# ssskkkky/EMME

Hardware: AMD Instinct MI355X
Metric: omega-points solved/sec (256-pt grid) (higher is better)
Workload: dtype f64

## Files before the change

### emme_amd/_lib.py

```python
from __future__ import annotations

import ctypes as C
import os

import numpy as np

HERE = os.path.dirname(os.path.abspath(__file__))
_LIB = None


class EmmeError(RuntimeError):
    def __init__(self, code, msg):
        super().__init__(f"[emme {code}] {msg}")
        self.code = code
        self.reason = msg


def lib_path() -> str:
    return os.environ.get("EMME_LIB") or os.path.join(HERE, "libemme_hip.so")


class Params(C.Structure):

    _fields_ = [
# ... 126 lines not shown
    lib.emme_ctx_set_options.argtypes = [P, C.POINTER(Options)]
    lib.emme_ctx_get_options.argtypes = [P, C.POINTER(Options)]
    lib.emme_null_vectors_batch.argtypes = [P, C.c_int, C.c_int, P, P, P]
    lib.emme_ctx_destroy.argtypes = [P]
    lib.emme_ctx_destroy.restype = None
    lib.emme_release_pooled_memory.argtypes = []
    lib.emme_release_pooled_memory.restype = None
    lib.emme_ctx_set_stream.argtypes = [P, P]
    lib.emme_ctx_set_tile_shapes.argtypes = [P, C.c_int]
    lib.emme_ctx_get_tile_shapes.argtypes = [P]
    lib.emme_ctx_set_deriv_cache_shapes.argtypes = [P, C.c_int]
    lib.emme_ctx_get_deriv_cache_shapes.argtypes = [P]
    if hasattr(lib, "emme_ctx_set_mirror_pairs"):
        lib.emme_ctx_set_mirror_pairs.argtypes = [P, C.c_int]
        lib.emme_ctx_get_mirror_pairs.argtypes = [P]
    lib.emme_ctx_dim.argtypes = [P]
    lib.emme_ctx_fill_mode.argtypes = [P]
    lib.emme_ctx_last_deferred.argtypes = [P]
    lib.emme_ctx_last_deferred.restype = C.c_longlong
    lib.emme_ctx_node_cache_gib.argtypes = [P]
    lib.emme_ctx_node_cache_gib.restype = C.c_double
    lib.emme_ctx_cache_settle.argtypes = [P, P, C.c_int, P]
    lib.emme_ctx_cache_state.argtypes = [P, P, P, P]
    lib.emme_ctx_profile_enable.argtypes = [P, C.c_int]
    lib.emme_ctx_profile_read.argtypes = [P, C.POINTER(Profile), C.c_int]
    lib.emme_assemble_batch.argtypes = [P, P, C.c_int, P, P]
    lib.emme_trace_solve_batch.argtypes = [P, C.c_int, C.c_int, P, P, P, P]
    lib.emme_qr_secant_batch.argtypes = [P, C.c_int, C.c_int, P, P, P, P]
    lib.emme_newton_step_batch.argtypes = [P, P, P, C.c_int, P, P, C.c_int, P]
    lib.emme_solve_roots.argtypes = [P, P, C.c_int, C.c_double, C.c_int, P, P, P, P]
# ... 364 lines not shown
    first = next((h for h in host if h is not None), None)
    nb, n = (first.shape[0], first.shape[1]) if first is not None else (int(A[0]), int(A[1]))
    for h in host:
        if h is not None and h.shape != (nb, n, n):
            raise ValueError("the operands must be [nbatch, n, n] of one shape")
    ptrs = [h.ctypes.data if h is not None else C.c_void_p(p) for h, p in zip(host, (a_device_ptr, b_device_ptr))]
    return ptrs[0], ptrs[1], nb, n, host


class Context:

    def __init__(self, params: Params, device: int = -1, **options):
        self.lib = load()
        self.params = params
        h = C.c_void_p()
        o = default_options(**options)
        _check(self.lib.emme_ctx_create_ex(C.byref(params), device, C.byref(o), C.byref(h)))
        self.h = h
        self.dim = self.lib.emme_ctx_dim(h)

    def options(self) -> Options:
        o = Options()
        _check(self.lib.emme_ctx_get_options(self.h, C.byref(o)))
        return o

    def set_options(self, **kw) -> None:
        o = self.options()
        for k, v in kw.items():
            if not hasattr(o, k):
                raise TypeError(f"unknown option {k!r}")
            setattr(o, k, v)
        _check(self.lib.emme_ctx_set_options(self.h, C.byref(o)))

    def set_tile_shapes(self, shapes: int) -> None:
# ... 4 lines not shown

    def deriv_cache_shapes(self) -> int:
        v = self.lib.emme_ctx_get_deriv_cache_shapes(self.h)
        if v < 0:
            _check(v)
        return v

    def tile_shapes(self) -> int:
        v = self.lib.emme_ctx_get_tile_shapes(self.h)
        if v < 0:
            _check(v)
        return v

    def set_mirror_pairs(self, on: bool) -> None:
        _check(self.lib.emme_ctx_set_mirror_pairs(self.h, 1 if on else 0))

    def mirror_pairs(self) -> int:
        v = self.lib.emme_ctx_get_mirror_pairs(self.h)
        if v < 0:
            _check(v)
        return v

    def close(self):
        if getattr(self, "h", None):
            self.lib.emme_ctx_destroy(self.h)
            self.h = None

    def __del__(self):
        try:
            self.close()
# ... 573 lines not shown
```

### emme_amd/csrc/ctx.hpp

```cpp
#pragma once
#include <hip/hip_runtime.h>

#include <algorithm>
#include <chrono>
#include <cmath>
#include <cstdio>
#include <cstdlib>
#include <cstring>
#include <functional>
#include <limits>
#include <mutex>
#include <string>
#include <vector>

#include "../../include/emme_hip.h"
#include "buffers.hpp"
#include "launch.hpp"
#include "options.hpp"
#include "pair_list.hpp"
#include "step_feedback.hpp"

namespace emme {

void set_error(const std::string& msg);
// ... 68 lines not shown
    emme_options_t opt{};
    int cache_depth = -1;
    NodeCacheGeom cache_geom{};
    int cache_max_intervals = 0;
    NodeCacheClass cache[2];
    bool em_shared = false;
    bool folded = true;
    bool tiled = false;
    DeviceBuffer<> d_btab;
    DeviceBuffer<> d_etab;
    DeviceBuffer<int> d_lu_items;
    DeviceBuffer<> d_lu_scratch;
    int n_cu = 256;
    int last_lu_nwg = 1;
    bool lu_one_wg = false;
    PinnedBuffer<int> p_act;
    PinnedBuffer<unsigned long long> p_iv;
    PinnedBuffer<double> p_w;
    PinnedBuffer<unsigned int> p_deferred;
    DeviceBuffer<unsigned int> d_overflow;
    PinnedBuffer<unsigned int> p_overflow;
    emme::StepFeedback fb;
    emme::StagingRing lists;
    bool ext_failed = false;
    DeviceBuffer<unsigned long long> d_defer_info;
    double cache_bytes_used = 0.0;
    DeviceBuffer<double> d_scale;
    DeviceBuffer<unsigned long long> d_worklist;
    DeviceBuffer<unsigned int> d_worklist_count;
    DeviceBuffer<unsigned long long> d_tile_worklist;
// ... 75 lines not shown
inline size_t batch_bytes(int n, int nbatch) { return (size_t)n * n * 2 * sizeof(double) * nbatch; }
int check_set_indices(const emme_ctx* c, const int* set, int n, const char* who);
int upload_set_indices(emme_ctx* c, const int* set, int n);
int ensure_batch(emme_ctx* c, int nb);
int ensure_mats(emme_ctx* c, int nb, int sets);
int upload_omega(emme_ctx* c, const double* omega, int n, hipMemcpyKind kind = hipMemcpyHostToDevice);
int reset_fill_counters(emme_ctx* c, int n);
int collect_fill_status(emme_ctx* c, int n, long long* intervals, int* bad_item = nullptr);
int queue_fill_counters(emme_ctx* c, int n, std::vector<unsigned long long>& iv, std::vector<int>* st);
int fold_fill_counters(emme_ctx* c, const std::vector<unsigned long long>& iv, const std::vector<int>* st,
                       long long* intervals = nullptr);

int check_method(const emme_ctx* c, int method);
hipError_t linear_step(emme_ctx* c, int method, int n, int nbatch, const double* M, double* work, double* Mp,
                       const int* active, double* tr, int* info, const int* h_active = nullptr, bool work_ready = false);
struct LuScratch {
    DeviceBuffer<double> b;
    DeviceBuffer<int> maps;
};
int lu_factor_batch(emme_ctx* c, int n, int nbatch, double* work, LuScratch& s, const char* who,
                    const std::function<hipError_t(int b0, int nb, const int* maps, int map_nb, const int* lu_info)>& after,
                    const int* d_items = nullptr, int nitems = 0);

struct AllocTimer {
    emme_ctx* c;
    std::chrono::steady_clock::time_point t0 = std::chrono::steady_clock::now();
    bool running = true;
    explicit AllocTimer(emme_ctx* ctx) : c(ctx) {}
    void stop() {
        if (running) {
// ... 32 lines not shown
```

### emme_amd/csrc/ctx_fill.hip

```cpp
#include "ctx.hpp"
#include "fill_plan.hpp"

namespace emme {

namespace {

FillShape shape_of(const emme_ctx* c, bool mirrored = false) {
    FillShape s;
    s.tiled = c->tiled, s.folded = c->folded;
    s.nm = c->nm, s.gk_points = c->p.integration_start_points, s.npairs = mirrored ? c->npairs_half : c->npairs;
    s.fill_lanes = c->opt.fill == EMME_FILL_LANES;
    s.dense_min_tasks = c->opt.dense_min_tasks, s.dense_cost_ratio = c->opt.dense_cost_ratio;
    s.union_ipg_few = c->opt.union_ipg_few, s.union_few_chunks = c->opt.union_few_chunks;
    return s;
}

bool deriv_shape_is_es15(const emme_ctx* c) { return c->nm == 1 && c->p.integration_start_points == 15; }
bool deriv_from_cache(const emme_ctx* c, const FillRequest& r) {
    return r.d_Md && c->opt.deriv_cached != 0 && c->tiled &&
           (deriv_shape_is_es15(c) || c->deriv_cache_shapes == EMME_DERIV_CACHE_SHAPES_ALL) && r.host_omega != nullptr;
}

bool runs_mirrored(const emme_ctx* c, const FillRequest& r, bool use_cache) {
    return c->mirror && c->tiled && use_cache && !r.d_Md && !r.d_set;
// ... 402 lines not shown
    ScopedSpan span(c, K_ASM);
    HIP_TRY((r.d_Md ? launch_assemble_sets_deriv : launch_assemble_sets)(L, c->d_sets, c->d_set_tabs, r.d_set, c->stream));
    return EMME_OK;
}

int fill_by_class(emme_ctx* c, const FillRequest& r, int minority) {
    std::vector<int> major(r.nbatch, 0), minor(r.nbatch, 0);
    for (int b : c->h_actidx) (contour_class(r.host_omega[2 * b]) == minority ? minor : major)[b] = 1;
    FillRequest part = r;
    part.host_active = major.data();
    EMME_TRY(fill(c, part));
    const int mode = c->last_fill_mode;
    part.host_active = minor.data(), part.force_uncached = true;
    const int rc = fill(c, part);
    c->last_fill_mode = mode;
    return rc;
}

}

int fill(emme_ctx* c, const FillRequest& r) {
    const bool has_wide = r.newton_loop && !r.d_Md && !r.d_set && c->tiled && c->nm == 1 && !c->fb.wide.empty();
    const int n_wide = plan_order(r.nbatch, r.host_active, r.cost, has_wide ? c->fb.wide.data() : nullptr, c->h_actidx);
    const int n_act = (int)c->h_actidx.size();
    if (n_act == 0) return EMME_OK;
    if (r.d_set) {
        AssembleLaunch L = make_launch(c, r, false);
        EMME_TRY(launch_sets(c, L, r));
        c->acc.matrices += n_act;
        return EMME_OK;
    }
    if (c->mirror && deriv_from_cache(c, r)) EMME_TRY(drop_mirror(c));
    bool use_cache = wants_cache(c, r);
    if (use_cache && !c->cache[0].recs && !c->cache[1].recs) c->mirror = mirror_wanted(c) && r.may_mirror;
    AssembleLaunch L = make_launch(c, r, runs_mirrored(c, r, use_cache));
    if (use_cache) {
        const bool has_cache[2] = {(bool)c->cache[0].recs, (bool)c->cache[1].recs};
        const ClassCensus classes = plan_classes(c->h_actidx, r.host_omega, has_cache);
        if (classes.minority >= 0) return fill_by_class(c, r, classes.minority);
        for (int k = 0; k < 2 && use_cache; ++k)
            if (classes.count[k] > 0) use_cache = ensure_node_cache(c, L, k);
        if (!use_cache && L.mirror) L = make_launch(c, r, false);
    }
    EMME_TRY(use_cache ? grow_cache_from_deferrals(c, L) : EMME_OK);
    EMME_TRY(use_cache ? fill_cached(c, L, r, n_wide) : fill_uncached(c, L, r));
    c->acc.matrices += n_act;
    return EMME_OK;
}

}
```

### emme_amd/csrc/ctx_linstep.hip

```cpp
#include "ctx.hpp"
#include "linstep_plan.hpp"

using namespace emme;

namespace {

hipError_t trace_solve(emme_ctx* c, int n, int nbatch, double* A, double* B, const int* active,
                       double* tr, int* info, const int* h_active) {
    const bool fits = trace_solve_blocked_lds(n) <= 150 * 1024;
    if (c->opt.lu_unblocked == 0 && (fits || n <= 1024)) {
        hipError_t e = c->d_lu_scratch.grow(trace_solve_blocked_scratch(n, nbatch));
        if (e != hipSuccess) return e;
        int n_live = nbatch;
        int* lu_slot = nullptr;
        if (h_active) {
            e = c->d_lu_items.grow(sizeof(int) * nbatch);
            if (e == hipSuccess) e = c->lists.take(nbatch, &lu_slot);
            if (e != hipSuccess) return e;
            n_live = 0;
            for (int b = 0; b < nbatch; ++b)
                if (h_active[b]) lu_slot[n_live++] = b;
            if (n_live == 0) return hipSuccess;
        }
        const int nwg = lu_workgroups(n, n_live, c->n_cu, c->opt.lu_split, c->lu_one_wg, fits);
// ... 46 lines not shown
    return EMME_OK;
}

hipError_t linear_step(emme_ctx* c, int method, int n, int nbatch, const double* M, double* work,
                       double* Mp, const int* active, double* tr, int* info, const int* h_active, bool work_ready) {
    if (method == EMME_METHOD_QR_SECANT) {
        hipError_t e = launch_transpose(n, nbatch, M, work, active, c->stream);
        if (e != hipSuccess) return e;
        return launch_qr_secant(n, nbatch, work, Mp, active, tr, info, c->stream);
    }
    if (!work_ready) {
        hipError_t e = hipMemcpyAsync(work, M, batch_bytes(n, nbatch), hipMemcpyDeviceToDevice, c->stream);
        if (e != hipSuccess) return e;
    }
    return trace_solve(c, n, nbatch, work, Mp, active, tr, info, h_active);
}

int lu_factor_batch(emme_ctx* c, int n, int nbatch, double* work, LuScratch& s, const char* who,
                    const std::function<hipError_t(int, int, const int*, int, const int*)>& after, const int* d_items,
                    int nitems) {
    const size_t mbytes = batch_bytes(n, 1);
    const bool one_wg = trace_solve_blocked_lds(n) <= 150 * 1024;
    const int todo = d_items ? nitems : nbatch;
    if (todo < 1) return EMME_OK;
    if (one_wg || (n <= 1024 && !(d_items && c->lu_one_wg))) {
        const int slice_max = one_wg ? todo : std::max(1, c->n_cu / 2);
        const int held = d_items ? nbatch : std::min(nbatch, slice_max);
        HIP_TRY(c->d_lu_scratch.grow(trace_solve_blocked_scratch(n, held)));
        if (!one_wg) HIP_TRY(s.b.grow(mbytes * held));
        for (int b0 = 0; b0 < todo; b0 += slice_max) {
// ... 97 lines not shown
    const size_t bytes = batch_bytes(n, nbatch);
    DeviceOperands ops;
    hipError_t staged = hipSuccess;
    EMME_TRY(ops.stage(c, A, B, bytes, &staged));
    HIP_TRY(staged);
    {
        ScopedSpan s(c, K_LIN);
        HIP_TRY(trace_solve(c, n, nbatch, ops.A, ops.B, nullptr, c->d_tr, c->d_info, nullptr));
    }
    HIP_TRY(hipMemcpyAsync(tr, c->d_tr, sizeof(double) * 2 * nbatch, hipMemcpyDeviceToHost, c->stream));
    HIP_TRY(hipMemcpyAsync(info, c->d_info, sizeof(int) * nbatch, hipMemcpyDeviceToHost, c->stream));
    HIP_TRY(hipStreamSynchronize(c->stream));
    return EMME_OK;
}

int emme_qr_secant_batch(emme_ctx_t* c, int n, int nbatch, const double* A, const double* B,
                         double* q, int* info) {
    if (!c || !A || !B || !q || !info || n < 1 || nbatch < 1) return EMME_EINVAL;
    if (n > 1024) {
        set_error("QR-secant step: matrix dimension above 1024 is not supported");
        return EMME_ECONFIG;
    }
    HIP_TRY(hipSetDevice(c->device));
    EMME_TRY(ensure_batch(c, nbatch));
    const size_t bytes = batch_bytes(n, nbatch);
    DeviceOperands ops;
    DeviceBuffer<double> dW;
    hipError_t e = hipSuccess;
    EMME_TRY(ops.stage(c, A, B, bytes, &e));
    if (e == hipErrorOutOfMemory || dW.grow(bytes) != hipSuccess) {
// ... 77 lines not shown
```

### emme_amd/csrc/ctx_search.hip

```cpp
#include "ctx.hpp"

using namespace emme;

namespace {

struct RootSearch {
    const double* guesses;
    int n;
    double tol;
    int step_limit;
    bool want_iterates;
    int method = 0;
    const int* set = nullptr;
    bool eigpair = false;
    const double* v0 = nullptr;
    LuScratch lu;
    std::vector<int> act, zeros;
    int stride() const { return step_limit + 1; }
    void to(const emme_ctx* c, FillRequest& r) const {
        if (set) r.d_set = c->d_set, r.host_set = set;
    }
    double* d_iterates(const emme_ctx* c) const { return want_iterates ? c->d_iterates.get() : nullptr; }
};

int search_begin(emme_ctx* c, RootSearch& s, int mat_sets) {
    const int n = s.n;
    EMME_TRY(ensure_batch(c, n));
    EMME_TRY(ensure_mats(c, n, mat_sets));
    if (s.want_iterates) {
        const size_t need = (size_t)n * s.stride() * 2;
        HIP_TRY(c->d_iterates.grow(need * sizeof(double)));
        std::vector<double> nanv(need, std::numeric_limits<double>::quiet_NaN());
        HIP_TRY(hipMemcpyAsync(c->d_iterates, nanv.data(), need * sizeof(double), hipMemcpyHostToDevice, c->stream));
        HIP_TRY(hipStreamSynchronize(c->stream));
    }
    s.act.assign(n, 1), s.zeros.assign(n, 0);
    if (s.set) EMME_TRY(upload_set_indices(c, s.set, n));
    if (s.eigpair) {
        const size_t vbytes = sizeof(double) * 2 * (size_t)n * c->dim;
        HIP_TRY(c->d_vecs.grow(vbytes));
        HIP_TRY(c->d_resid.grow(sizeof(double) * n));
        HIP_TRY(c->p_live.grow(sizeof(int) * n));
        if (s.v0) HIP_TRY(hipMemcpyAsync(c->d_vecs, s.v0, vbytes, hipMemcpyHostToDevice, c->stream));
    }
    HIP_TRY(hipMemcpyAsync(c->d_active, s.act.data(), sizeof(int) * n, hipMemcpyHostToDevice, c->stream));
    HIP_TRY(hipMemcpyAsync(c->d_iters, s.zeros.data(), sizeof(int) * n, hipMemcpyHostToDevice, c->stream));
    HIP_TRY(hipMemcpyAsync(c->d_info, s.zeros.data(), sizeof(int) * n, hipMemcpyHostToDevice, c->stream));
    return reset_fill_counters(c, n);
}

int search_end(emme_ctx* c, const RootSearch& s, double* roots, int* iters, int* info, double* iterates, bool* repeat) {
// ... 64 lines not shown
    StepFeedback& fb = c->fb;
    fb.begin(n);
    HIP_TRY(hipMemsetAsync(c->d_overflow, 0, sizeof(unsigned int) * n, c->stream));
    std::vector<double> h_w(2 * (size_t)n);
    std::vector<unsigned long long> iv_now(n, 0), iv_prev_dbg(n, 0);
    auto refresh_cost = [&]() -> int {
        HIP_TRY(hipMemcpyAsync(iv_now.data(), c->d_intervals, sizeof(unsigned long long) * n, hipMemcpyDeviceToHost, c->stream));
        HIP_TRY(hipStreamSynchronize(c->stream));
        fb.take(iv_now.data());
        return EMME_OK;
    };
    FillRequest first(n, c->d_omega, c->d_Mold);
    first.host_omega = w0.data(), first.newton_loop = true;
    search.to(c, first);
    EMME_TRY(fill(c, first));
    EMME_TRY(refresh_cost());
    HIP_TRY(hipMemcpyAsync(c->d_omega, w1.data(), sizeof(double) * 2 * n, hipMemcpyHostToDevice, c->stream));
    FillRequest next(n, c->d_omega, c->d_M);
    next.host_omega = w1.data(), next.cost = fb.cost.data(), next.newton_loop = true;
    search.to(c, next);
    EMME_TRY(fill(c, next));
    next.host_omega = h_w.data(), next.d_active = c->d_active, next.host_active = act.data();

    EMME_TRY(refresh_cost());
    bool pending = false;
    int j_pending = 0;
    auto take_pending = [&]() {
        std::copy(c->p_act.get(), c->p_act.get() + n, act.begin());
        fb.take(c->p_iv, c->p_overflow, cache_npairs(c), c->p_deferred);
        pending = false;
        if (std::getenv("EMME_DEBUG")) {
            unsigned long long tot = 0, mx = 0;
            int na = 0, nprev = 0;
            for (int b = 0; b < n; ++b) {
                if (fb.iv_prev[b] != iv_prev_dbg[b]) {
                    const unsigned long long d = fb.iv_prev[b] - iv_prev_dbg[b];
// ... 7 lines not shown
                    j_pending, nprev, tot, mx, na);
        }
    };
    const bool eig = search.eigpair;
    if (eig) std::fill(c->p_live.get(), c->p_live.get() + n, 1);
    for (int j = 0; j <= step_limit; ++j) {
        const bool fused_copy = method == EMME_METHOD_TRACE_SECANT;
        if (eig) {
            {
                ScopedSpan s(c, K_LIN);
                HIP_TRY(launch_copy_active(c->dim, n, c->d_M, c->d_work, nullptr, c->d_active, c->stream));
            }
            EMME_TRY(eigpair_step(c, search, c->p_live.get(), j == 0 && !search.v0, true));
            ScopedSpan s(c, K_OTHER);
            HIP_TRY(launch_copy_active(c->dim, n, c->d_M, c->d_Mold, nullptr, c->d_active, c->stream));
        } else {
            {
                ScopedSpan s(c, K_OTHER);
                HIP_TRY(launch_secant_copy_sym(c->dim, n, c->d_M, c->d_Mold, fused_copy ? c->d_work : nullptr, c->d_Mp,
                                               c->d_domega, c->d_active, c->stream));
            }
            ScopedSpan s(c, K_LIN);
            HIP_TRY(linear_step(c, method, c->dim, n, c->d_M, c->d_work, c->d_Mp, c->d_active, c->d_tr, c->d_info,
                                act.data(), fused_copy));
        }
        {
            ScopedSpan s(c, K_OTHER);
            HIP_TRY(launch_newton_update(n, c->d_tr, c->d_omega, c->d_domega, c->d_active, c->d_iters,
                                         c->d_info, tol, d_iterates, j, stride, c->stream, c->p_w,
                                         c->opt.skip_lost ? c->d_status : nullptr));
        }
        if (eig) HIP_TRY(hipMemcpyAsync(c->p_live, c->d_active, sizeof(int) * n, hipMemcpyDeviceToHost, c->stream));
        HIP_TRY(hipStreamSynchronize(c->stream));
        std::copy(c->p_w.get(), c->p_w.get() + 2 * (size_t)n, h_w.begin());
        if (pending) {
            take_pending();
            bool any = false;
            for (int b = 0; b < n; ++b) any |= act[b] != 0;
            if (!any) break;
        }
        EMME_TRY(fill(c, next));
        {
            ScopedSpan s(c, K_OTHER);
            HIP_TRY(launch_retire(n, c->d_active, c->stream, c->p_act, c->d_intervals, c->p_iv,
                                  c->d_worklist_count, c->p_deferred, c->d_overflow, c->p_overflow));
        }
        pending = true, j_pending = j;
    }
    if (eig) {
        ScopedSpan s(c, K_LIN);
        HIP_TRY(launch_eigpair_resid(c->dim, c->d_M, nullptr, n, c->d_vecs, c->d_resid, c->stream));
    }
    return EMME_OK;
}

int newton_loop(emme_ctx* c, RootSearch& search) {
// ... 227 lines not shown
```

### emme_amd/csrc/emme_capi.hip

```cpp
#include "ctx.hpp"

namespace emme {

static thread_local std::string g_error;
void set_error(const std::string& msg) { g_error = msg; }

bool is_device_ptr(const void* p) {
    if (!p) return false;
    hipPointerAttribute_t attr;
    hipError_t e = hipPointerGetAttributes(&attr, p);
    if (e != hipSuccess) {
        (void)hipGetLastError();
        return false;
    }
    return attr.type == hipMemoryTypeDevice;
}

hipEvent_t get_event(emme_ctx* c) {
    if (!c->free_events.empty()) {
        hipEvent_t e = c->free_events.back();
        c->free_events.pop_back();
        return e;
    }
    hipEvent_t e;
// ... 252 lines not shown
    c->em_shared = !es && o.em_shared != 0;
    c->folded = o.phase_table != 0;
    c->tiled = wants_tiled(*p, c->folded, o.fill);

    DevParams& P = c->P;
    std::vector<double> tab;
    dev_params_from(p, P, tab);

    std::vector<PairIJ> pairs, half;
    full_pair_list(N, pairs);
    half_pair_list(N, half);
    c->npairs = (int)pairs.size();
    c->npairs_half = (int)half.size();
    c->mirror_ok = c->nm == 1 && p->integration_start_points == 15 && grid_is_mirror_symmetric(tab.data(), N, 1e-13);
    if (const char* v = std::getenv("EMME_MIRROR")) c->mirror_opt = std::atoi(v) != 0;

    auto fail = [&](int code) {
        emme_ctx_destroy(c);
        return code;
    };
    if (c->d_tab.grow(tab.size() * sizeof(double)) != hipSuccess ||
        c->d_pairs.grow(pairs.size() * sizeof(ushort2)) != hipSuccess ||
        c->d_pairs_half.grow(half.size() * sizeof(ushort2)) != hipSuccess) {
        set_error("hipMalloc failed for tables");
        return fail(EMME_ENOMEM);
    }
    if (hipMemcpy(c->d_tab, tab.data(), tab.size() * sizeof(double), hipMemcpyHostToDevice) != hipSuccess ||
        hipMemcpy(c->d_pairs, pairs.data(), pairs.size() * sizeof(ushort2), hipMemcpyHostToDevice) != hipSuccess ||
        hipMemcpy(c->d_pairs_half, half.data(), half.size() * sizeof(ushort2), hipMemcpyHostToDevice) != hipSuccess) {
        set_error("hipMemcpy failed for tables");
// ... 65 lines not shown
        set_error("emme_ctx_set_mirror_pairs: value out of range (0, 1)");
        return EMME_EINVAL;
    }
    if (c->cache[0].recs || c->cache[1].recs) {
        set_error("emme_ctx_set_mirror_pairs: the pair list fixes the layout of the node cache, which exists already");
        return EMME_EINVAL;
    }
    c->mirror_opt = on;
    return EMME_OK;
}

int emme_ctx_get_mirror_pairs(const emme_ctx_t* c) {
    if (!c) return EMME_EINVAL;
    return (c->cache[0].recs || c->cache[1].recs) ? (int)c->mirror : (int)mirror_wanted(c);
}

int emme_ctx_set_deriv_cache_shapes(emme_ctx_t* c, int shapes) {
    if (!c) {
        set_error("emme_ctx_set_deriv_cache_shapes: NULL context");
        return EMME_EINVAL;
    }
    if (shapes != EMME_DERIV_CACHE_SHAPES_ES15 && shapes != EMME_DERIV_CACHE_SHAPES_ALL) {
        set_error("emme_ctx_set_deriv_cache_shapes: value out of range (EMME_DERIV_CACHE_SHAPES_ES15, EMME_DERIV_CACHE_SHAPES_ALL)");
        return EMME_EINVAL;
    }
    c->deriv_cache_shapes = shapes;
    return EMME_OK;
}

int emme_ctx_get_deriv_cache_shapes(const emme_ctx_t* c) { return c ? c->deriv_cache_shapes : EMME_EINVAL; }
// ... 200 lines not shown
```

### emme_amd/csrc/launch.hpp

```cpp
#pragma once
#include <hip/hip_runtime.h>

#include "emme_device.hpp"

namespace emme {

constexpr int NODE_CACHE_MAX_SUB = 12;
struct NodeCacheGeom {
    int dfull;
    int nsub;
    int rd[NODE_CACHE_MAX_SUB], dd[NODE_CACHE_MAX_SUB];
    unsigned long long rp[NODE_CACHE_MAX_SUB];
};
struct AssembleLaunch {
    DevParams P;
    int gk_points;
    int nbatch;
    int npairs;
    int items_per_group;
    const double* tab;
    const void* pairs;
    const double* omega;
    const int* active;
    double* M;
// ... 140 lines not shown
                              const int* active, hipStream_t stream);

hipError_t launch_secant_copy(int n, int nbatch, const double* M, double* Mold, double* work, double* Mp,
                              const double* domega, const int* active, hipStream_t stream);

hipError_t launch_secant_copy_sym(int n, int nbatch, const double* M, double* Mold, double* work, double* Mp,
                                  const double* domega, const int* active, hipStream_t stream);

size_t trace_solve_blocked_lds(int n);
size_t trace_solve_chunked_lds(int n);
size_t trace_solve_blocked_scratch(int n, int nbatch);
hipError_t launch_trace_solve_blocked(int n, int nbatch, double* A, double* B, const int* active,
                                      double* tr, int* info, int nwg, const int* items, int nitems,
                                      void* scratch, hipStream_t stream, int group_min_n = 256, int spin_limit = 0);

hipError_t launch_lu_inplace(int n, int nbatch, double* A, const int* items, int nitems, int* info, void* scratch,
                             hipStream_t stream);
int trace_solve_nb();
const int* trace_solve_rowmaps(const void* scratch, int n, int nbatch);
hipError_t launch_lu_unblocked_inplace(int n, int nbatch, double* A, int* maps, int* info, hipStream_t stream,
                                       const int* items = nullptr, int nitems = 0);
size_t null_iterate_lds(int n);
hipError_t launch_null_iterate(int n, const double* A_lu, const int* rowmaps, int nb, const int* items, int nitems,
                               const int* lu_info, double* vecs, int* info, int max_sweeps, hipStream_t stream);

hipError_t launch_eigpair_step(int n, const double* M, const double* Mp, const double* A_lu, const int* rowmaps, int nb,
                               const int* items, int nitems, const int* active, const int* lu_info, double* vecs,
                               double* tau, double* resid, int* info, bool first, hipStream_t stream);
hipError_t launch_eigpair_secant_step(int n, const double* M, const double* Mold, const double* domega, const double* A_lu,
                                      const int* rowmaps, int nb, const int* items, int nitems, const int* active,
// ... 59 lines not shown
```

### include/emme_hip.h

```cpp
#ifndef EMME_HIP_H
#define EMME_HIP_H

#include <stddef.h>

#include "emme_params.h"

#ifdef __cplusplus
extern "C" {
#endif

#define EMME_OK 0
#define EMME_EINVAL (-1)
#define EMME_EJSON (-2)
#define EMME_EDEVICE (-3)
#define EMME_ENOMEM (-4)
#define EMME_ECONFIG (-5)
#define EMME_ENUMERIC (-6)

typedef struct emme_ctx emme_ctx_t;

typedef struct emme_profile {
    double assemble_ms;
    long assemble_launches;
    double deferred_ms;
// ... 64 lines not shown
int emme_ctx_create_ex(const emme_params_t* p, int device, const emme_options_t* opt, emme_ctx_t** out);
int emme_ctx_set_options(emme_ctx_t* ctx, const emme_options_t* opt);
int emme_ctx_get_options(const emme_ctx_t* ctx, emme_options_t* opt);
void emme_ctx_destroy(emme_ctx_t* ctx);
void emme_release_pooled_memory(void);
#define EMME_TILE_SHAPES_ES15 0
#define EMME_TILE_SHAPES_ALL  1
int emme_ctx_set_tile_shapes(emme_ctx_t* ctx, int shapes);
int emme_ctx_get_tile_shapes(const emme_ctx_t* ctx);
#define EMME_DERIV_CACHE_SHAPES_ES15 0
#define EMME_DERIV_CACHE_SHAPES_ALL  1
int emme_ctx_set_deriv_cache_shapes(emme_ctx_t* ctx, int shapes);
int emme_ctx_get_deriv_cache_shapes(const emme_ctx_t* ctx);
int emme_ctx_set_mirror_pairs(emme_ctx_t* ctx, int on);
int emme_ctx_get_mirror_pairs(const emme_ctx_t* ctx);
int emme_ctx_set_stream(emme_ctx_t* ctx, void* hip_stream);
int emme_ctx_dim(const emme_ctx_t* ctx);
int emme_ctx_fill_mode(const emme_ctx_t* ctx);
long long emme_ctx_last_deferred(emme_ctx_t* ctx);
double emme_ctx_node_cache_gib(const emme_ctx_t* ctx);
int emme_ctx_cache_settle(emme_ctx_t* ctx, const double* omega, int nbatch, int* fills_done);
int emme_ctx_cache_state(const emme_ctx_t* ctx, int* full_depth, int* subtrees, double* gib);
int emme_ctx_profile_enable(emme_ctx_t* ctx, int on);
int emme_ctx_profile_read(emme_ctx_t* ctx, emme_profile_t* out, int reset);

int emme_assemble_batch(emme_ctx_t* ctx, const double* omega, int nbatch, double* M,
                        long long* intervals);

int emme_newton_step_batch(emme_ctx_t* ctx, double* omega, double* domega, int nbatch,
                           double* M, double* Mp, int method, int* info);

int emme_trace_solve_batch(emme_ctx_t* ctx, int n, int nbatch, double* A, double* B, double* tr,
                           int* info);

int emme_qr_secant_batch(emme_ctx_t* ctx, int n, int nbatch, const double* A, const double* B,
                         double* q, int* info);

int emme_solve_roots(emme_ctx_t* ctx, const double* guesses, int n, double tol, int step_limit,
                     double* roots, int* iters, int* info, double* iterates);
int emme_assemble_derivative_batch(emme_ctx_t* ctx, const double* omega, int nbatch, double* M, double* Mp,
                                   long long* intervals);
int emme_solve_roots_newton(emme_ctx_t* ctx, const double* guesses, int n, double tol, int step_limit,
                            double* roots, int* iters, int* info, double* iterates);
int emme_params_same_shape(const emme_params_t* a, const emme_params_t* b);
int emme_ctx_bind_param_sets(emme_ctx_t* ctx, const emme_params_t* sets, int nsets);
int emme_ctx_param_sets(const emme_ctx_t* ctx);
int emme_assemble_sets_batch(emme_ctx_t* ctx, const int* set, const double* omega, int nbatch,
                             double* M, double* Mp, long long* intervals);
// ... 116 lines not shown
```

Before: 30530.

## Fold mirror-symmetric secant step into two half-size LU solves with rank correction

Measured after the change: 32010, median of 6. 4.8% higher.

```diff
diff --git a/emme_amd/_lib.py b/emme_amd/_lib.py
--- a/emme_amd/_lib.py
+++ b/emme_amd/_lib.py
@@ -164,6 +164,11 @@
     if hasattr(lib, "emme_ctx_set_mirror_pairs"):
         lib.emme_ctx_set_mirror_pairs.argtypes = [P, C.c_int]
         lib.emme_ctx_get_mirror_pairs.argtypes = [P]
+    if hasattr(lib, "emme_ctx_set_lu_fold"):
+        lib.emme_ctx_set_lu_fold.argtypes = [P, C.c_int]
+        lib.emme_ctx_get_lu_fold.argtypes = [P]
+        lib.emme_ctx_last_folded_steps.argtypes = [P]
+        lib.emme_trace_secant_folded_batch.argtypes = [P, C.c_int, C.c_int, P, P, P, P, P]
     lib.emme_ctx_dim.argtypes = [P]
     lib.emme_ctx_fill_mode.argtypes = [P]
     lib.emme_ctx_last_deferred.argtypes = [P]
@@ -558,10 +563,13 @@
         self.lib = load()
         self.params = params
         h = C.c_void_p()
+        lu_fold = options.pop("lu_fold", None)
         o = default_options(**options)
         _check(self.lib.emme_ctx_create_ex(C.byref(params), device, C.byref(o), C.byref(h)))
         self.h = h
         self.dim = self.lib.emme_ctx_dim(h)
+        if lu_fold is not None:
+            self.set_lu_fold(lu_fold)
 
     def options(self) -> Options:
         o = Options()
@@ -596,6 +604,34 @@
 
     def set_mirror_pairs(self, on: bool) -> None:
         _check(self.lib.emme_ctx_set_mirror_pairs(self.h, 1 if on else 0))
+
+    def set_lu_fold(self, on) -> None:
+        _check(self.lib.emme_ctx_set_lu_fold(self.h, int(on)))
+
+    def lu_fold(self) -> int:
+        v = self.lib.emme_ctx_get_lu_fold(self.h)
+        if v < 0:
+            _check(v)
+        return v
+
+    def last_folded_steps(self) -> int:
+        return self.lib.emme_ctx_last_folded_steps(self.h)
+
+    def trace_secant_folded(self, M, M_old, domega, device_ptrs=None):
+        if device_ptrs is not None:
+            nb, n = int(M[0]), int(M[1])
+            _check(self.lib.emme_trace_secant_folded_batch(self.h, n, nb, *[C.c_void_p(int(p)) for p in device_ptrs]))
+            return None
+        M = _c128(M)
+        M = np.ascontiguousarray(M[None] if M.ndim == 2 else M)
+        Mo = _c128(M_old, M.shape)
+        nb, n = M.shape[0], M.shape[1]
+        dw = _c128(np.broadcast_to(np.asarray(domega, dtype=np.complex128), (nb,)))
+        tr = np.zeros(nb, dtype=np.complex128)
+        info = np.zeros(nb, dtype=np.int32)
+        _check(self.lib.emme_trace_secant_folded_batch(self.h, n, nb, M.ctypes.data, Mo.ctypes.data, dw.ctypes.data,
+                                                       tr.ctypes.data, info.ctypes.data))
+        return tr, info
 
     def mirror_pairs(self) -> int:
         v = self.lib.emme_ctx_get_mirror_pairs(self.h)
diff --git a/emme_amd/csrc/ctx.hpp b/emme_amd/csrc/ctx.hpp
--- a/emme_amd/csrc/ctx.hpp
+++ b/emme_amd/csrc/ctx.hpp
@@ -106,6 +106,14 @@
     int n_cu = 256;
     int last_lu_nwg = 1;
     bool lu_one_wg = false;
+    int lu_fold = 1;
+    bool last_fill_mirrored = false;
+    int last_folded_steps = 0;
+    struct FoldScratch {
+        DeviceBuffer<double> vecs, tr2, part;
+        DeviceBuffer<int> act2, info2, lu_info, items;
+        DeviceBuffer<> lu_scratch;
+    } fold;
     PinnedBuffer<int> p_act;
     PinnedBuffer<unsigned long long> p_iv;
     PinnedBuffer<double> p_w;
@@ -211,6 +219,9 @@
 int check_method(const emme_ctx* c, int method);
 hipError_t linear_step(emme_ctx* c, int method, int n, int nbatch, const double* M, double* work, double* Mp,
                        const int* active, double* tr, int* info, const int* h_active = nullptr, bool work_ready = false);
+bool fold_applies(const emme_ctx* c, int n);
+int folded_secant_step(emme_ctx* c, int n, int nbatch, const double* M, const double* Mold, double* Mold_w, double* work,
+                       double* Mp, const double* domega, const int* active, double* tr, int* info, const int* h_active);
 struct LuScratch {
     DeviceBuffer<double> b;
     DeviceBuffer<int> maps;
diff --git a/emme_amd/csrc/ctx_fill.hip b/emme_amd/csrc/ctx_fill.hip
--- a/emme_amd/csrc/ctx_fill.hip
+++ b/emme_amd/csrc/ctx_fill.hip
@@ -440,6 +440,7 @@
     part.host_active = minor.data(), part.force_uncached = true;
     const int rc = fill(c, part);
     c->last_fill_mode = mode;
+    c->last_fill_mirrored = false;
     return rc;
 }
 
@@ -449,6 +450,7 @@
     const bool has_wide = r.newton_loop && !r.d_Md && !r.d_set && c->tiled && c->nm == 1 && !c->fb.wide.empty();
     const int n_wide = plan_order(r.nbatch, r.host_active, r.cost, has_wide ? c->fb.wide.data() : nullptr, c->h_actidx);
     const int n_act = (int)c->h_actidx.size();
+    c->last_fill_mirrored = false;
     if (n_act == 0) return EMME_OK;
     if (r.d_set) {
         AssembleLaunch L = make_launch(c, r, false);
@@ -470,6 +472,7 @@
     }
     EMME_TRY(use_cache ? grow_cache_from_deferrals(c, L) : EMME_OK);
     EMME_TRY(use_cache ? fill_cached(c, L, r, n_wide) : fill_uncached(c, L, r));
+    c->last_fill_mirrored = use_cache && L.mirror != 0;
     c->acc.matrices += n_act;
     return EMME_OK;
 }
diff --git a/emme_amd/csrc/ctx_linstep.hip b/emme_amd/csrc/ctx_linstep.hip
--- a/emme_amd/csrc/ctx_linstep.hip
+++ b/emme_amd/csrc/ctx_linstep.hip
@@ -84,6 +84,57 @@
         if (e != hipSuccess) return e;
     }
     return trace_solve(c, n, nbatch, work, Mp, active, tr, info, h_active);
+}
+
+bool fold_applies(const emme_ctx* c, int n) {
+    return c->lu_fold != 0 && n >= 2 && n % 2 == 0 && c->opt.lu_unblocked == 0 &&
+           trace_solve_blocked_lds(n / 2) <= 150 * 1024 && null_iterate_lds(n / 2) <= 150 * 1024;
+}
+
+int folded_secant_step(emme_ctx* c, int n, int nbatch, const double* M, const double* Mold, double* Mold_w, double* work,
+                       double* Mp, const double* domega, const int* active, double* tr, int* info, const int* h_active) {
+    const int m = n / 2, nhalf = 2 * nbatch;
+    emme_ctx::FoldScratch& f = c->fold;
+    HIP_TRY(f.vecs.grow(sizeof(double) * 2 * 4 * (size_t)m * nbatch));
+    HIP_TRY(f.tr2.grow(sizeof(double) * 2 * nhalf));
+    HIP_TRY(f.part.grow(fold_part_bytes(nbatch)));
+    HIP_TRY(f.act2.grow(sizeof(int) * nhalf));
+    HIP_TRY(f.info2.grow(sizeof(int) * nhalf));
+    HIP_TRY(f.lu_info.grow(sizeof(int) * nhalf));
+    HIP_TRY(f.lu_scratch.grow(trace_solve_blocked_scratch(m, nhalf)));
+    const size_t second = (size_t)nbatch * n * n;
+    double *S1 = work, *S2 = work + second, *D1 = Mp, *D2 = Mp + second;
+    {
+        ScopedSpan s(c, K_OTHER);
+        HIP_TRY(launch_fold_edges(n, nbatch, M, Mold, domega, active, f.vecs, f.act2, c->stream));
+        HIP_TRY(launch_fold_pass(n, nbatch, M, Mold, Mold_w, S1, S2, D1, D2, domega, active, c->stream));
+    }
+    std::vector<int> h2;
+    const int* d_items = nullptr;
+    int n_live = nhalf;
+    if (h_active) {
+        h2.resize(nhalf);
+        int* slot = nullptr;
+        HIP_TRY(f.items.grow(sizeof(int) * nhalf));
+        HIP_TRY(c->lists.reserve(nhalf));
+        HIP_TRY(c->lists.take(nhalf, &slot));
+        n_live = 0;
+        for (int b = 0; b < nbatch; ++b) {
+            h2[2 * b] = h2[2 * b + 1] = h_active[b] != 0;
+            if (h_active[b]) slot[n_live++] = 2 * b, slot[n_live++] = 2 * b + 1;
+        }
+        if (n_live == 0) return EMME_OK;
+        HIP_TRY(launch_stage_ints(slot, f.items, n_live, nullptr, 0, c->stream));
+        HIP_TRY(c->lists.read_on(c->stream));
+        d_items = f.items;
+    }
+    ScopedSpan s(c, K_LIN);
+    HIP_TRY(launch_lu_inplace(m, nhalf, S2, d_items, n_live, f.lu_info, f.lu_scratch, c->stream));
+    HIP_TRY(trace_solve(c, m, nhalf, S1, D1, f.act2, f.tr2, f.info2, h_active ? h2.data() : nullptr));
+    HIP_TRY(launch_fold_solve(m, S2, trace_solve_rowmaps(f.lu_scratch, m, nhalf), trace_solve_nb(), d_items, n_live,
+                              f.lu_info, D2, f.vecs, f.part, c->stream));
+    HIP_TRY(launch_fold_combine(n, nbatch, active, f.tr2, f.info2, f.lu_info, f.part, tr, info, c->stream));
+    return EMME_OK;
 }
 
 int lu_factor_batch(emme_ctx* c, int n, int nbatch, double* work, LuScratch& s, const char* who,
@@ -211,6 +262,54 @@
     return EMME_OK;
 }
 
+int emme_trace_secant_folded_batch(emme_ctx_t* c, int n, int nbatch, const double* M, const double* M_old,
+                                   const double* domega, double* tr, int* info) {
+    const char* who = "emme_trace_secant_folded_batch";
+    if (!c || !M || !M_old || !domega || !tr || !info || n < 1 || nbatch < 1) {
+        set_error(std::string(who) + ": a required pointer is NULL, n < 1 or nbatch < 1");
+        return EMME_EINVAL;
+    }
+    if (n % 2 != 0) {
+        set_error(std::string(who) + ": the order must be even");
+        return EMME_EINVAL;
+    }
+    if (trace_solve_blocked_lds(n / 2) > 150 * 1024 || null_iterate_lds(n / 2) > 150 * 1024 || c->opt.lu_unblocked != 0) {
+        set_error(std::string(who) + ": the half problems need the blocked one-workgroup kernels (order above 1050, or lu_unblocked)");
+        return EMME_ECONFIG;
+    }
+    const void* sides[5] = {M, M_old, domega, tr, info};
+    bool dev = false;
+    EMME_TRY(same_side_all(sides, 5, "M, M_old, domega, tr and info", &dev));
+    HIP_TRY(hipSetDevice(c->device));
+    EMME_TRY(ensure_batch(c, 2 * nbatch));
+    const size_t bytes = batch_bytes(n, nbatch), cb = sizeof(double) * 2 * nbatch, ib = sizeof(int) * nbatch;
+    DeviceBuffer<double> t_m, t_old, t_dw, t_work, t_mp, t_tr;
+    DeviceBuffer<int> t_info;
+    HIP_TRY(t_work.grow(bytes));
+    HIP_TRY(t_mp.grow(bytes));
+    const double *dM = M, *dOld = M_old, *dDw = domega;
+    double* dTr = tr;
+    int* dInfo = info;
+    if (!dev) {
+        HIP_TRY(t_m.grow(bytes));
+        HIP_TRY(t_old.grow(bytes));
+        HIP_TRY(t_dw.grow(cb));
+        HIP_TRY(t_tr.grow(cb));
+        HIP_TRY(t_info.grow(ib));
+        HIP_TRY(hipMemcpyAsync(t_m, M, bytes, hipMemcpyHostToDevice, c->stream));
+        HIP_TRY(hipMemcpyAsync(t_old, M_old, bytes, hipMemcpyHostToDevice, c->stream));
+        HIP_TRY(hipMemcpyAsync(t_dw, domega, cb, hipMemcpyHostToDevice, c->stream));
+        dM = t_m, dOld = t_old, dDw = t_dw, dTr = t_tr, dInfo = t_info;
+    }
+    EMME_TRY(folded_secant_step(c, n, nbatch, dM, dOld, nullptr, t_work, t_mp, dDw, nullptr, dTr, dInfo, nullptr));
+    if (!dev) {
+        HIP_TRY(hipMemcpyAsync(tr, t_tr, cb, hipMemcpyDeviceToHost, c->stream));
+        HIP_TRY(hipMemcpyAsync(info, t_info, ib, hipMemcpyDeviceToHost, c->stream));
+    }
+    HIP_TRY(hipStreamSynchronize(c->stream));
+    return EMME_OK;
+}
+
 int emme_qr_secant_batch(emme_ctx_t* c, int n, int nbatch, const double* A, const double* B,
                          double* q, int* info) {
     if (!c || !A || !B || !q || !info || n < 1 || nbatch < 1) return EMME_EINVAL;
diff --git a/emme_amd/csrc/ctx_search.hip b/emme_amd/csrc/ctx_search.hip
--- a/emme_amd/csrc/ctx_search.hip
+++ b/emme_amd/csrc/ctx_search.hip
@@ -35,6 +35,7 @@
         HIP_TRY(hipStreamSynchronize(c->stream));
     }
     s.act.assign(n, 1), s.zeros.assign(n, 0);
+    c->last_folded_steps = 0;
     if (s.set) EMME_TRY(upload_set_indices(c, s.set, n));
     if (s.eigpair) {
         const size_t vbytes = sizeof(double) * 2 * (size_t)n * c->dim;
@@ -129,12 +130,14 @@
     first.host_omega = w0.data(), first.newton_loop = true;
     search.to(c, first);
     EMME_TRY(fill(c, first));
+    bool old_mirrored = c->last_fill_mirrored, new_mirrored = false;
     EMME_TRY(refresh_cost());
     HIP_TRY(hipMemcpyAsync(c->d_omega, w1.data(), sizeof(double) * 2 * n, hipMemcpyHostToDevice, c->stream));
     FillRequest next(n, c->d_omega, c->d_M);
     next.host_omega = w1.data(), next.cost = fb.cost.data(), next.newton_loop = true;
     search.to(c, next);
     EMME_TRY(fill(c, next));
+    new_mirrored = c->last_fill_mirrored;
     next.host_omega = h_w.data(), next.d_active = c->d_active, next.host_active = act.data();
 
     EMME_TRY(refresh_cost());
@@ -172,6 +175,10 @@
             EMME_TRY(eigpair_step(c, search, c->p_live.get(), j == 0 && !search.v0, true));
             ScopedSpan s(c, K_OTHER);
             HIP_TRY(launch_copy_active(c->dim, n, c->d_M, c->d_Mold, nullptr, c->d_active, c->stream));
+        } else if (fused_copy && c->mirror && old_mirrored && new_mirrored && fold_applies(c, c->dim)) {
+            EMME_TRY(folded_secant_step(c, c->dim, n, c->d_M, c->d_Mold, c->d_Mold, c->d_work, c->d_Mp, c->d_domega,
+                                        c->d_active, c->d_tr, c->d_info, act.data()));
+            ++c->last_folded_steps;
         } else {
             {
                 ScopedSpan s(c, K_OTHER);
@@ -197,7 +204,9 @@
             for (int b = 0; b < n; ++b) any |= act[b] != 0;
             if (!any) break;
         }
+        old_mirrored = new_mirrored;
         EMME_TRY(fill(c, next));
+        new_mirrored = c->last_fill_mirrored;
         {
             ScopedSpan s(c, K_OTHER);
             HIP_TRY(launch_retire(n, c->d_active, c->stream, c->p_act, c->d_intervals, c->p_iv,
diff --git a/emme_amd/csrc/emme_capi.hip b/emme_amd/csrc/emme_capi.hip
--- a/emme_amd/csrc/emme_capi.hip
+++ b/emme_amd/csrc/emme_capi.hip
@@ -290,6 +290,7 @@
     c->npairs_half = (int)half.size();
     c->mirror_ok = c->nm == 1 && p->integration_start_points == 15 && grid_is_mirror_symmetric(tab.data(), N, 1e-13);
     if (const char* v = std::getenv("EMME_MIRROR")) c->mirror_opt = std::atoi(v) != 0;
+    if (const char* v = std::getenv("EMME_LU_FOLD")) c->lu_fold = std::atoi(v) != 0;
 
     auto fail = [&](int code) {
         emme_ctx_destroy(c);
@@ -385,6 +386,23 @@
     if (!c) return EMME_EINVAL;
     return (c->cache[0].recs || c->cache[1].recs) ? (int)c->mirror : (int)mirror_wanted(c);
 }
+
+int emme_ctx_set_lu_fold(emme_ctx_t* c, int on) {
+    if (!c) {
+        set_error("emme_ctx_set_lu_fold: NULL context");
+        return EMME_EINVAL;
+    }
+    if (on != 0 && on != 1) {
+        set_error("emme_ctx_set_lu_fold: value out of range (0, 1)");
+        return EMME_EINVAL;
+    }
+    c->lu_fold = on;
+    return EMME_OK;
+}
+
+int emme_ctx_get_lu_fold(const emme_ctx_t* c) { return c ? c->lu_fold : EMME_EINVAL; }
+
+int emme_ctx_last_folded_steps(const emme_ctx_t* c) { return c ? c->last_folded_steps : EMME_EINVAL; }
 
 int emme_ctx_set_deriv_cache_shapes(emme_ctx_t* c, int shapes) {
     if (!c) {
diff --git a/emme_amd/csrc/launch.hpp b/emme_amd/csrc/launch.hpp
--- a/emme_amd/csrc/launch.hpp
+++ b/emme_amd/csrc/launch.hpp
@@ -178,6 +178,16 @@
                                       double* tr, int* info, int nwg, const int* items, int nitems,
                                       void* scratch, hipStream_t stream, int group_min_n = 256, int spin_limit = 0);
 
+hipError_t launch_fold_edges(int n, int nbatch, const double* M, const double* Mold, const double* domega,
+                             const int* active, double* vecs, int* act2, hipStream_t stream);
+hipError_t launch_fold_pass(int n, int nbatch, const double* M, const double* Mold, double* Mold_w, double* S1, double* S2,
+                            double* D1, double* D2, const double* domega, const int* active, hipStream_t stream);
+size_t fold_part_bytes(int nbatch);
+hipError_t launch_fold_solve(int m, const double* S_lu, const int* rowmaps, int nb, const int* items, int nitems,
+                             const int* lu_info, const double* Sp, const double* vecs, double* part, hipStream_t stream);
+hipError_t launch_fold_combine(int n, int nbatch, const int* active, const double* tr2, const int* info2, const int* lu_info,
+                               const double* part, double* tr, int* info, hipStream_t stream);
+
 hipError_t launch_lu_inplace(int n, int nbatch, double* A, const int* items, int nitems, int* info, void* scratch,
                              hipStream_t stream);
 int trace_solve_nb();
diff --git a/emme_amd/csrc/linstep_fold.hip b/emme_amd/csrc/linstep_fold.hip
--- /dev/null
+++ b/emme_amd/csrc/linstep_fold.hip
@@ -0,0 +1,287 @@
+#include <hip/hip_runtime.h>
+
+#include "emme_device.hpp"
+#include "launch.hpp"
+#include "tri_solve.hpp"
+
+namespace emme {
+
+namespace {
+
+using namespace trisolve;
+
+constexpr int FT = 32;
+
+__device__ __forceinline__ cd ldc(const double2* p) {
+    const double2 v = *p;
+    return mk(v.x, v.y);
+}
+__device__ __forceinline__ double2 d2(cd v) { return make_double2(v.x, v.y); }
+
+__device__ __forceinline__ cd edge_u(const double2* X, int n, int k) {
+    if (k == n - 1) return 0.5 * (ldc(&X[(size_t)(n - 1) * n + n - 1]) - ldc(&X[0]));
+    return ldc(&X[(size_t)k * n + n - 1]) - ldc(&X[n - 1 - k]);
+}
+
+__global__ __launch_bounds__(256) void k_fold_edges(int n, const double2* M, const double2* Mold, const double2* domega,
+                                                    const int* active, double2* vecs, int* act2) {
+    const int b = blockIdx.x;
+    const int live = active ? active[b] != 0 : 1;
+    if (threadIdx.x == 0) act2[2 * b] = live, act2[2 * b + 1] = live;
+    if (!live) return;
+    const int m = n / 2;
+    const cd rdw = rcp(mk(domega[b].x, domega[b].y));
+    const double2* X = M + (size_t)b * n * n;
+    const double2* O = Mold + (size_t)b * n * n;
+    double2* v = vecs + (size_t)b * 4 * m;
+    for (int i = threadIdx.x; i < m; i += 256) {
+        const int i2 = n - 1 - i;
+        const cd u1 = edge_u(X, n, i), u2 = edge_u(X, n, i2);
+        const cd d1 = (u1 - edge_u(O, n, i)) * rdw, dd2 = (u2 - edge_u(O, n, i2)) * rdw;
+        v[i] = d2(u1 + u2), v[m + i] = d2(u1 - u2);
+        v[2 * m + i] = d2(d1 + dd2), v[3 * m + i] = d2(d1 - dd2);
+    }
+}
+
+__global__ __launch_bounds__(256) void k_fold_pass(int n, int nfold, const double2* M, const double2* Mold, double2* Mold_w,
+                                                   double2* S1, double2* S2, double2* D1, double2* D2,
+                                                   const double2* domega, const int* active) {
+    const int b = blockIdx.y;
+    if (active && active[b] == 0) return;
+    __shared__ double2 s_p[FT][FT + 1], s_m[FT][FT + 1];
+    const int m = n / 2;
+    const size_t base = (size_t)b * n * n;
+    const int tx = threadIdx.x & (FT - 1), ty = threadIdx.x / FT;
+    const bool copy_tile = (int)blockIdx.x >= nfold;
+    const int nt = ((copy_tile ? n : m) + FT - 1) / FT;
+    int I = 0, rem = copy_tile ? blockIdx.x - nfold : blockIdx.x;
+    while (rem >= nt - I) rem -= nt - I, ++I;
+    const int J = I + rem;
+    if (copy_tile) {
+        if (I * FT + J * FT + 2 * (FT - 1) <= n - 1) return;
+        for (int rr = ty; rr < FT; rr += 256 / FT) {
+            const int r = I * FT + rr, c = J * FT + tx;
+            if (r < n && c < n && r <= c && c > n - 1 - r) Mold_w[base + (size_t)r * n + c] = M[base + (size_t)r * n + c];
+        }
+        return;
+    }
+    const cd rdw = rcp(mk(domega[b].x, domega[b].y));
+    cd dp[FT / 8], dm[FT / 8];
+#pragma unroll
+    for (int q = 0; q < FT / 8; ++q) {
+        const int rr = ty + 8 * q;
+        const int i = I * FT + rr, j = J * FT + tx;
+        cd sp = mk(0.0, 0.0), sm = sp;
+        dp[q] = sp, dm[q] = sp;
+        if (i < m && j < m && (I != J || rr <= tx)) {
+            const size_t ip = base + (size_t)i * n + j, iq = base + (size_t)i * n + (n - 1 - j);
+            const double2 vp = M[ip], vq = M[iq];
+            const cd P = mk(vp.x, vp.y), Q = mk(vq.x, vq.y);
+            const cd Pd = (P - ldc(&Mold[ip])) * rdw, Qd = (Q - ldc(&Mold[iq])) * rdw;
+            if (Mold_w) Mold_w[ip] = vp, Mold_w[iq] = vq;
+            sp = P + Q, sm = P - Q;
+            dp[q] = Pd + Qd, dm[q] = Pd - Qd;
+        }
+        s_p[rr][tx] = d2(sp), s_m[rr][tx] = d2(sm);
+    }
+    auto write_out = [&](double2* out1, double2* out2) {
+        double2* p1 = out1 + (size_t)(2 * b) * m * m;
+        double2* p2 = out2 + (size_t)(2 * b) * m * m;
+        const size_t minus = (size_t)m * m;
+        for (int rr = ty; rr < FT; rr += 256 / FT) {
+            const int r = I * FT + rr, c = J * FT + tx;
+            if (r < m && c < m) {
+                const bool lower = I == J && rr > tx;
+                const size_t idx = (size_t)r * m + c;
+                const double2 vp = lower ? s_p[tx][rr] : s_p[rr][tx], vm = lower ? s_m[tx][rr] : s_m[rr][tx];
+                p1[idx] = vp, p2[idx] = vp, p1[minus + idx] = vm, p2[minus + idx] = vm;
+            }
+        }
+        if (I != J) {
+            for (int rr = ty; rr < FT; rr += 256 / FT) {
+                const int r = J * FT + rr, c = I * FT + tx;
+                if (r < m && c < m) {
+                    const size_t idx = (size_t)r * m + c;
+                    const double2 vp = s_p[tx][rr], vm = s_m[tx][rr];
+                    p1[idx] = vp, p2[idx] = vp, p1[minus + idx] = vm, p2[minus + idx] = vm;
+                }
+            }
+        }
+    };
+    __syncthreads();
+    write_out(S1, S2);
+    __syncthreads();
+#pragma unroll
+    for (int q = 0; q < FT / 8; ++q) s_p[ty + 8 * q][tx] = d2(dp[q]), s_m[ty + 8 * q][tx] = d2(dm[q]);
+    __syncthreads();
+    write_out(D1, D2);
+}
+
+constexpr int NPART = 9;
+
+struct FoldSolveArgs {
+    int m, nb, nblk;
+    const double2* A;
+    const int* maps;
+    const int* items;
+    const int* lu_info;
+    const double2* D;
+    const double2* vecs;
+    double2* part;
+};
+
+__global__ __launch_bounds__(NT) void k_fold_solve(FoldSolveArgs P) {
+    extern __shared__ double2 sm[];
+    __shared__ double s_red[6 * NW];
+    const int m = P.m;
+    double2* x0 = sm;
+    double2* xa = sm + m;
+    double2* xb = sm + 2 * (size_t)m;
+    int* rowmap = reinterpret_cast<int*>(sm + 3 * (size_t)m);
+    const int h = P.items ? P.items[blockIdx.x] : blockIdx.x;
+    const int tid = threadIdx.x, lane = tid & 63, wave = tid >> 6;
+    double2* out = P.part + (size_t)h * NPART;
+    if (P.lu_info[h] != 0) {
+        const double qnan = __builtin_nan("");
+        if (tid < NPART) out[tid] = make_double2(qnan, qnan);
+        return;
+    }
+    const double sgn = (h & 1) ? -1.0 : 1.0;
+    const double2* u = P.vecs + ((size_t)(h >> 1) * 4 + (h & 1)) * m;
+    const double2* ud = u + 2 * (size_t)m;
+    Factors F;
+    F.n = m, F.a = P.A + (size_t)h * m * m, F.rowmap = rowmap;
+    F.bA = sm + 3 * (size_t)m + rowmap_slots(m);
+    F.bD = F.bA + 2 * TB * (TB + 1);
+    const int* maps = P.maps + (size_t)h * P.nblk * m;
+    for (int x = tid; x < m; x += NT) rowmap[x] = maps[(size_t)(x / P.nb) * m + x], x0[x] = u[x];
+    __syncthreads();
+    solve_plain(F, x0, xa);
+    for (int x = tid; x < m; x += NT) x0[x] = make_double2(x == 0 ? sgn : 0.0, 0.0);
+    __syncthreads();
+    solve_plain(F, x0, xb);
+    const double2* D = P.D + (size_t)h * m * m;
+    cd fba = mk(0.0, 0.0), faa = fba, fbb = fba;
+    for (int r = wave; r < m; r += NW) {
+        const double2* row = D + (size_t)r * m;
+        cd ya = mk(0.0, 0.0), yb = ya;
+        for (int c = lane; c < m; c += 64) {
+            const cd d = ldc(&row[c]);
+            ya = ya + d * mk(xa[c].x, xa[c].y);
+            yb = yb + d * mk(xb[c].x, xb[c].y);
+        }
+        ya.x = wave_sum(ya.x), ya.y = wave_sum(ya.y), yb.x = wave_sum(yb.x), yb.y = wave_sum(yb.y);
+        const cd ar = mk(xa[r].x, xa[r].y), br = mk(xb[r].x, xb[r].y);
+        fba = fba + br * ya, faa = faa + ar * ya, fbb = fbb + br * yb;
+    }
+    auto block_sum6 = [&](const double (&v)[6], double (&t)[6]) {
+        __syncthreads();
+        if (lane == 0)
+            for (int q = 0; q < 6; ++q) s_red[q * NW + wave] = v[q];
+        __syncthreads();
+        for (int q = 0; q < 6; ++q) {
+            t[q] = 0.0;
+            for (int k = 0; k < NW; ++k) t[q] += s_red[q * NW + k];
+        }
+    };
+    double t[6];
+    {
+        const double v[6] = {fba.x, fba.y, faa.x, faa.y, fbb.x, fbb.y};
+        block_sum6(v, t);
+    }
+    if (tid == 0) {
+        out[6] = make_double2(t[0], t[1]), out[7] = make_double2(t[2], t[3]), out[8] = make_double2(t[4], t[5]);
+        out[0] = make_double2(sgn * xa[0].x, sgn * xa[0].y), out[1] = make_double2(sgn * xb[0].x, sgn * xb[0].y);
+    }
+    cd ua = mk(0.0, 0.0), ub = ua, da = ua, db = ua;
+    for (int x = tid; x < m; x += NT) {
+        const cd a = mk(xa[x].x, xa[x].y), bb = mk(xb[x].x, xb[x].y), uu = ldc(&u[x]), dd = ldc(&ud[x]);
+        ua = ua + uu * a, ub = ub + uu * bb, da = da + dd * a, db = db + dd * bb;
+    }
+    {
+        const double v[6] = {wave_sum(ua.x), wave_sum(ua.y), wave_sum(ub.x), wave_sum(ub.y), wave_sum(da.x), wave_sum(da.y)};
+        block_sum6(v, t);
+    }
+    if (tid == 0) out[2] = make_double2(t[0], t[1]), out[3] = make_double2(t[2], t[3]), out[4] = make_double2(t[4], t[5]);
+    {
+        const double v[6] = {wave_sum(db.x), wave_sum(db.y), 0.0, 0.0, 0.0, 0.0};
+        block_sum6(v, t);
+    }
+    if (tid == 0) out[5] = make_double2(t[0], t[1]);
+}
+
+__global__ void k_fold_combine(int n, int nbatch, const int* active, const double2* tr2, const int* info2,
+                               const int* lu_info, const double2* part, double2* tr, int* info) {
+    const int b = blockIdx.x * blockDim.x + threadIdx.x;
+    if (b >= nbatch) return;
+    if (active && active[b] == 0) return;
+    const int m = n / 2;
+    int inf = 0;
+    for (int s = 1; s >= 0; --s) {
+        const int i2 = info2[2 * b + s] != 0 ? info2[2 * b + s] : lu_info[2 * b + s];
+        if (i2 != 0) inf = i2 > 0 ? i2 + s * m : i2;
+    }
+    const double2* pp = part + (size_t)(2 * b) * NPART;
+    const double2* pm = pp + NPART;
+    auto both = [&](int q) { return 0.5 * (mk(pp[q].x, pp[q].y) + mk(pm[q].x, pm[q].y)); };
+    const cd ea = both(0), eb = both(1), ua = both(2), ub = both(3), au = both(4), bu = both(5);
+    const cd fba = both(6), faa = both(7), fbb = both(8);
+    const cd g11 = fba + bu * ea + eb * au;
+    const cd g12 = fbb + 2.0 * (bu * eb);
+    const cd g21 = faa + 2.0 * (au * ea);
+    const cd k11 = mk(1.0, 0.0) + ea, k12 = eb, k21 = ua, k22 = mk(1.0, 0.0) + ub;
+    const cd det = k11 * k22 - k12 * k21;
+    if (inf == 0 && !((det.x != 0.0 || det.y != 0.0) && isfinite(det.x) && isfinite(det.y))) inf = n + 1;
+    const cd trkg = (k22 * g11 - k12 * g21 - k21 * g12 + k11 * g11) * rcp(det);
+    const cd t = mk(tr2[2 * b].x, tr2[2 * b].y) + mk(tr2[2 * b + 1].x, tr2[2 * b + 1].y) + 2.0 * bu - trkg;
+    const double qnan = __builtin_nan("");
+    tr[b] = inf != 0 ? make_double2(qnan, qnan) : make_double2(t.x, t.y);
+    info[b] = inf;
+}
+
+}
+
+size_t fold_part_bytes(int nbatch) { return sizeof(double2) * NPART * 2 * (size_t)nbatch; }
+
+hipError_t launch_fold_edges(int n, int nbatch, const double* M, const double* Mold, const double* domega,
+                             const int* active, double* vecs, int* act2, hipStream_t stream) {
+    hipLaunchKernelGGL(k_fold_edges, dim3(nbatch), dim3(256), 0, stream, n, (const double2*)M, (const double2*)Mold,
+                       (const double2*)domega, active, (double2*)vecs, act2);
+    return hipGetLastError();
+}
+
+hipError_t launch_fold_pass(int n, int nbatch, const double* M, const double* Mold, double* Mold_w, double* S1, double* S2,
+                            double* D1, double* D2, const double* domega, const int* active, hipStream_t stream) {
+    const int m = n / 2;
+    const int ntm = (m + FT - 1) / FT, ntn = (n + FT - 1) / FT;
+    const int nfold = ntm * (ntm + 1) / 2, ncopy = Mold_w ? ntn * (ntn + 1) / 2 : 0;
+    hipLaunchKernelGGL(k_fold_pass, dim3((unsigned)(nfold + ncopy), nbatch), dim3(256), 0, stream, n, nfold,
+                       (const double2*)M, (const double2*)Mold, (double2*)Mold_w, (double2*)S1, (double2*)S2, (double2*)D1,
+                       (double2*)D2, (const double2*)domega, active);
+    return hipGetLastError();
+}
+
+hipError_t launch_fold_solve(int m, const double* S_lu, const int* rowmaps, int nb, const int* items, int nitems,
+                             const int* lu_info, const double* Sp, const double* vecs, double* part, hipStream_t stream) {
+    FoldSolveArgs P;
+    P.m = m, P.nb = nb, P.nblk = (m + nb - 1) / nb;
+    P.A = (const double2*)S_lu, P.maps = rowmaps, P.items = items, P.lu_info = lu_info;
+    P.D = (const double2*)Sp, P.vecs = (const double2*)vecs, P.part = (double2*)part;
+    const size_t lds = null_iterate_lds(m);
+    if (lds > 150 * 1024) return hipErrorNotSupported;
+    if (lds > 48 * 1024) {
+        const hipError_t ea = hipFuncSetAttribute((const void*)k_fold_solve, hipFuncAttributeMaxDynamicSharedMemorySize, (int)lds);
+        if (ea != hipSuccess) return ea;
+    }
+    hipLaunchKernelGGL(k_fold_solve, dim3(nitems), dim3(NT), lds, stream, P);
+    return hipGetLastError();
+}
+
+hipError_t launch_fold_combine(int n, int nbatch, const int* active, const double* tr2, const int* info2, const int* lu_info,
+                               const double* part, double* tr, int* info, hipStream_t stream) {
+    hipLaunchKernelGGL(k_fold_combine, dim3((nbatch + 63) / 64), dim3(64), 0, stream, n, nbatch, active, (const double2*)tr2,
+                       info2, lu_info, (const double2*)part, (double2*)tr, info);
+    return hipGetLastError();
+}
+
+}
diff --git a/include/emme_hip.h b/include/emme_hip.h
--- a/include/emme_hip.h
+++ b/include/emme_hip.h
@@ -102,6 +102,9 @@
 int emme_ctx_get_deriv_cache_shapes(const emme_ctx_t* ctx);
 int emme_ctx_set_mirror_pairs(emme_ctx_t* ctx, int on);
 int emme_ctx_get_mirror_pairs(const emme_ctx_t* ctx);
+int emme_ctx_set_lu_fold(emme_ctx_t* ctx, int on);
+int emme_ctx_get_lu_fold(const emme_ctx_t* ctx);
+int emme_ctx_last_folded_steps(const emme_ctx_t* ctx);
 int emme_ctx_set_stream(emme_ctx_t* ctx, void* hip_stream);
 int emme_ctx_dim(const emme_ctx_t* ctx);
 int emme_ctx_fill_mode(const emme_ctx_t* ctx);
@@ -120,6 +123,9 @@
 
 int emme_trace_solve_batch(emme_ctx_t* ctx, int n, int nbatch, double* A, double* B, double* tr,
                            int* info);
+
+int emme_trace_secant_folded_batch(emme_ctx_t* ctx, int n, int nbatch, const double* M, const double* M_old,
+                                   const double* domega, double* tr, int* info);
 
 int emme_qr_secant_batch(emme_ctx_t* ctx, int n, int nbatch, const double* A, const double* B,
                          double* q, int* info);
```
